# boromir674/relation-autoencoder

Hardware: AMD Instinct MI355X
Metric: train examples/sec (fwd+bwd) K=100 d=200 neg=20 at 1/2/4/8 MI355X (higher is better)
Workload: dtype fp32

## Files before the change

relation-autoencoder_amd/csrc/rae.hip:

```cpp
#include <hip/hip_runtime.h>
#include <hip/hip_ext.h>

#include <algorithm>
#include <cmath>
#include <cstdlib>
#include <cstdio>
#include <cstring>
#include <string>
#include <type_traits>

#include "../../include/rae.h"
#include "rae_bilinear.hpp"
#include "rae_cluster.hpp"
#include "rae_sp_split.hpp"
#include "rae_common.hpp"
#include "rae_dp.hpp"
#include "rae_eval.hpp"
#include "rae_index.hpp"
#include "rae_label.hpp"
#include "rae_p2p.hpp"
#include "rae_profile.hpp"
#include "rae_rank.hpp"
#include "rae_topk.hpp"
#include "rae_sampler.hpp"
// ... 493 lines not shown
    __shared__ double red[RAE_EV_NW * RAE_RK_NSUM];
    rank_blocksum(greater, equal, target, lse, n, hk, partial, red);
}
__global__ void k_rank_acc(const double* partial, int nblk, double* summary, int init) {
    const int c = threadIdx.x;
    if (blockIdx.x != 0 || c >= RAE_RK_NSUM) return;
    double t = init ? 0.0 : summary[c];
    for (int b = 0; b < nblk; ++b) t += partial[b * RAE_RK_NSUM + c];
    summary[c] = t;
}

template <bool AV4>
__global__ __launch_bounds__(RAE_RK_BT) void k_topk(RankArgs a, TopkOut o) {
    extern __shared__ __attribute__((aligned(16))) char smem[];
    topk_scores<AV4>(a, o, smem);
}
__global__ __launch_bounds__(RAE_ETK_FQ * 64) void k_topk_finish(const rae_key64* keys, int strips,
                                                                  int nq, int top, int32_t* ents,
                                                                  float* scores) {
    __shared__ rae_key64 sList[RAE_ETK_FQ * 32];
    topk_finish(keys, strips, nq, top, ents, scores, sList);
}

__global__ void k_add_cursor(int64_t* cursor, int64_t count) {
    if (threadIdx.x == 0 && blockIdx.x == 0) *cursor += count;
}
__global__ void k_set_cursor(int64_t* cursor, int64_t v) {
    if (threadIdx.x == 0 && blockIdx.x == 0) *cursor = v;
}

static thread_local std::string g_last_error;

static int fail(int code, const std::string& msg) {
    g_last_error = msg;
    return code;
}
#define HIPCHK(x)                                                                          \
    do {                                                                                   \
        hipError_t e_ = (x);                                                               \
        if (e_ != hipSuccess)                                                              \
            return fail(RAE_E_HIP, std::string(#x) + ": " + hipGetErrorString(e_));       \
    } while (0)

struct rae_plan : PlanSpec {
    rae_config cfg;
    rae_buffers buf;
    int64_t cursor_moves = 0;
    int* h_err = nullptr;
    unsigned* d_sig = nullptr;
    bool peers_set = false;
    int peers_mask = 0;
    char* ws = nullptr;
    unsigned long long* stamps_fwd = nullptr;
    unsigned long long* stamps_upd = nullptr;
    hipEvent_t t_start = nullptr, t_stop = nullptr;
};

#define RAE_LAUNCH(p, K, g, b, sh, st, ...)                                                 \
    do {                                                                                  \
        if ((p)->t_stop) {                                                                \
            hipEvent_t e0_ = (p)->t_start;                                                \
            (p)->t_start = nullptr;                                                       \
            hipExtLaunchKernelGGL(K, g, b, sh, st, e0_, (p)->t_stop, 0, __VA_ARGS__);      \
        } else {                                                                          \
            hipLaunchKernelGGL(K, g, b, sh, st, __VA_ARGS__);                             \
        }                                                                                 \
    } while (0)

#define RAE_CV(x) decltype(x)::value
template <class F> static void with_bool(bool b, F&& f) {
    if (b) f(std::true_type{}); else f(std::false_type{});
}
template <class F> static void with_q(int q, F&& f) {
    if (q == 1) f(std::integral_constant<int, 1>{}); else f(std::integral_constant<int, 2>{});
}
template <class F> static void with_opt(int opt, F&& f) {
    if (opt == RAE_OPT_ADAGRAD) f(std::integral_constant<int, 0>{});
    else f(std::integral_constant<int, 1>{});
}

extern "C" const char* rae_last_error(void) { return g_last_error.c_str(); }
extern "C" int rae_version(void) { return RAE_VERSION; }
#ifndef RAE_BUILD_ID
#define RAE_BUILD_ID "unversioned"
#endif
#ifdef RAE_DIAG
#define RAE_BUILD_KIND "diag-"
#else
#define RAE_BUILD_KIND ""
#endif
__attribute__((used)) static const char g_build_id[] = "RAE_BUILD_ID:" RAE_BUILD_KIND RAE_BUILD_ID;
extern "C" const char* rae_build_id(void) { return g_build_id + 13; }

extern "C" int64_t rae_exchange_record_floats(const rae_config* cfg) {
    if (!cfg) return -1;
    return plan_layout(*cfg).rec;
}
extern "C" int64_t rae_exchange_floats(const rae_config* cfg) {
    if (!cfg) return -1;
    return rae_exchange_record_floats(cfg) * (int64_t)cfg->batch_size * cfg->world_size;
}

static void plan_set_kernel_attributes(const rae_plan* p) {
    auto lds = [](const void* f, size_t bytes) {
        (void)hipFuncSetAttribute(f, hipFuncAttributeMaxDynamicSharedMemorySize, (int)bytes);
    };
// ... 140 lines not shown

static void launch_fwd_dp(rae_plan* p, const StepArgs& a, hipStream_t st);
template <bool V4>
static void launch_fwd_bil(rae_plan* p, const StepArgs& a, hipStream_t st) {
    const dim3 ge(p->grid_fwd);
    if (V4 && a.dec == RAE_DEC_RESCAL && a.m == 100 && a.r == 200 && a.s == 20)
        RAE_LAUNCH(p, (k_bil_enc_fast<DimsC3>), ge, dim3(RAE_FBT), p->smem_fwd, st, a);
    else
        RAE_LAUNCH(p, (k_bil_enc<V4>), ge, dim3(RAE_FBT), p->smem_fwd, st, a);
    const dim3 gmt(((a.r + RAE_MTI - 1) / RAE_MTI) * ((a.r + RAE_MTJ - 1) / RAE_MTJ));
    for (int pass = 0; pass < 2; ++pass) {
        if (pass == 1) RAE_LAUNCH(p, (k_bil_dec<V4>), ge, dim3(RAE_DBT), p->smem_dec, st, a);
        if (p->mt_bf16 && pass == 0)
            RAE_LAUNCH(p, (k_bil_mt<true, false, false>), gmt, dim3(RAE_MTT), p->smem_mt0, st, a, pass);
        else if (p->mt_bf16) RAE_LAUNCH(p, (k_bil_mt<true>), gmt, dim3(RAE_MTT), p->smem_mt, st, a, pass);
        else if (p->mt_direct) RAE_LAUNCH(p, (k_bil_mt<false, true>), gmt, dim3(RAE_MTT), 0, st, a, pass);
        else RAE_LAUNCH(p, (k_bil_mt<false>), gmt, dim3(RAE_MTT), p->smem_mt, st, a, pass);
    }
    if (!a.mtP) launch_fwd_dp(p, a, st);
    RAE_LAUNCH(p, k_bil_fin, ge, dim3(RAE_FINT), 0, st, a);
}

static void launch_fwd_dp(rae_plan* p, const StepArgs& a, hipStream_t st) {
    const int gd = ceil_div(bil_dp_tasks(a.l, a.m, a.nib), RAE_NWAVE);
    const size_t lds77 = dp2_lds_bytes<7, 7>(), lds88 = dp2_lds_bytes<8, 8>();
    if (p->dp2 == 1)
        RAE_LAUNCH(p, (k_bil_dp2<7, 7>), dim3(a.nib), dim3(dp2_threads<7, 7>()), lds77, st, a);
    else if (p->dp2 == 2)
        RAE_LAUNCH(p, (k_bil_dp2<8, 8>), dim3(a.nib), dim3(dp2_threads<8, 8>()), lds88, st, a);
    else
        with_bool(a.bf16, [&](auto B) { RAE_LAUNCH(p, k_bil_dp<RAE_CV(B)>, dim3(gd), dim3(RAE_BT), 0, st, a); });
}

static unsigned p2p_rows_grid(const StepArgs& a) {
    const int64_t g = ((int64_t)a.G * (a.capA + a.capW) + RAE_NWAVE - 1) / RAE_NWAVE;
    return (unsigned)(g < 1 ? 1 : g);
}
static unsigned p2p_recs_grid(const StepArgs& a) {
    const int64_t g = ((int64_t)a.l * a.lay.rec / 4 + RAE_BT - 1) / RAE_BT;
    return (unsigned)(g < 1 ? 1 : g);
}
static bool p2p_on(const rae_plan* p) { return p->args.xchg != RAE_XCHG_COLLECTIVE && p->args.G > 1; }
static int p2p_pre_mark_blocks(const StepArgs& a) {
    const int64_t n = (int64_t)a.G * (a.capA + a.capW);
    return (int)((n + RAE_BT - 1) / RAE_BT);
}

static int launch_forward(rae_plan* p, const int64_t* cursor, int64_t off, hipStream_t st) {
    if (!p->args.neg1 || !p->args.neg2) return fail(RAE_E_STATE, "negatives not set");
    StepArgs a = p->args;
    a.cursor = cursor;
    a.step_offset = off;
    a.stamps = p->stamps_fwd;
    const bool p2p = p2p_on(p);
    if (p2p) {
        if (!p->peers_set) return fail(RAE_E_STATE, "peer buffers not set (rae_set_peer)");
        if (!a.pipe) {
            const unsigned gr = p2p_rows_grid(a);
            RAE_LAUNCH(p, k_p2p_rows, dim3(gr), dim3(RAE_BT), 0, st, a);
            RAE_LAUNCH(p, k_p2p_signal, dim3(1), dim3(64), 0, st, a, 1);
        }
        RAE_LAUNCH(p, k_p2p_wait, dim3(1), dim3(64), 0, st, a, 1, 1u);
    }
    if (a.dec == RAE_DEC_SP) {
        launch_fwd_sp(p, a, st);
        if (a.dpart)
            RAE_LAUNCH(p, k_dpart, dim3(dpart_tasks(a.r, a.m)), dim3(RAE_BT), 0, st, a);
    }
    else with_bool(p->v4, [&](auto V) { launch_fwd_bil<RAE_CV(V)>(p, a, st); });
    if (p2p)
    {
        RAE_LAUNCH(p, k_p2p_recs, dim3(p2p_recs_grid(a) + (a.pipe ? 64 : 0)), dim3(RAE_BT), 0, st, a);
        RAE_LAUNCH(p, k_p2p_signal, dim3(1), dim3(64), 0, st, a, 0);
        if (a.pipe) {
            const int nmb = p2p_pre_mark_blocks(a);
            RAE_LAUNCH(p, k_p2p_pre, dim3(nmb + p2p_rows_grid(a)), dim3(RAE_BT), 0, st, a, 0, nmb);
        }
    }
    p->t_start = p->t_stop = nullptr;
    HIPCHK(hipGetLastError());
    return RAE_OK;
}

template <int OPT, bool V4, bool BIL>
static void launch_update_b(rae_plan* p, dim3 gu, dim3 bt, hipStream_t st, const StepArgs& a) {
    if constexpr (BIL) {
        if (a.bf16 && !a.fuse_prep) {
            const int gp = 4 * ((a.r + 63) / 64) * (a.Lp / 32) + (a.Lp / 32) * ((a.m + 15) / 16);
            RAE_LAUNCH(p, k_bil_prep, dim3(gp), bt, 0, st, a);
        }
        const int nRt = n_rtiles(a.dec, a.r, a.m);
        const dim3 gr((nRt + RAE_NWAVE - 1) / RAE_NWAVE);
        const size_t lr = bil_rows_lds_bytes(a.m, a.bf16, OPT == 0);
        constexpr size_t lu = 4 * update_lds_floats<V4, 2>();
        if (RAE_BIL_FUSED_UPD && lr >= lu) {
            const dim3 gf(gu.x + gr.x);
            with_bool(a.pipe, [&](auto PP) { with_q(p->q, [&](auto Q) {
                RAE_LAUNCH(p, (k_bil_update<OPT, V4, RAE_CV(Q), RAE_CV(PP)>), gf, bt, lr, st, a, (int)gu.x);
            }); });
            return;
        }
        with_bool(lr != 0, [&](auto LDS) {
            RAE_LAUNCH(p, (k_bil_rows<OPT, RAE_CV(LDS)>), gr, bt, lr, st, a);
        });
        with_bool(a.pipe, [&](auto PP) { with_q(p->q, [&](auto Q) {
            RAE_LAUNCH(p, (k_update_bil<OPT, V4, RAE_CV(Q), RAE_CV(PP)>), gu, bt, 0, st, a);
// ... 306 lines not shown

extern "C" int rae_time_next(rae_plan* p, void* start, void* stop) {
    if (!p) return fail(RAE_E_INVALID, "null plan");
    if (!start || !stop) return fail(RAE_E_INVALID, "null event");
    p->t_start = (hipEvent_t)start;
    p->t_stop = (hipEvent_t)stop;
    return RAE_OK;
}
extern "C" int rae_event_create(void** ev) {
    if (!ev) return fail(RAE_E_INVALID, "null argument");
    hipEvent_t e = nullptr;
    HIPCHK(hipEventCreate(&e));
    *ev = (void*)e;
    return RAE_OK;
}
extern "C" int rae_event_destroy(void* ev) {
    if (ev) HIPCHK(hipEventDestroy((hipEvent_t)ev));
    return RAE_OK;
}
extern "C" int rae_event_elapsed_ms(void* start, void* stop, float* ms) {
    if (!start || !stop || !ms) return fail(RAE_E_INVALID, "null argument");
    HIPCHK(hipEventSynchronize((hipEvent_t)stop));
    HIPCHK(hipEventElapsedTime(ms, (hipEvent_t)start, (hipEvent_t)stop));
    return RAE_OK;
}

extern "C" int rae_train_step(rae_plan* p, int64_t batch, const int32_t* n1, const int32_t* n2,
                              rae_stream_t stream) {
    if (!p) return fail(RAE_E_INVALID, "null plan");
    if (p->cfg.world_size != 1)
        return fail(RAE_E_STATE, "rae_train_step is the single-rank func['train'] path");
    const int64_t nb = p->cfg.n_examples / p->cfg.batch_size;
    if (batch < 0 || batch >= nb) return fail(RAE_E_INVALID, "batch index out of range");
    int rc = rae_set_negatives(p, n1, n2, RAE_NEG_PER_CALL, p->cfg.batch_size);
    if (rc) return rc;
    rc = launch_index(p, batch, 1, (hipStream_t)stream);
    if (rc) return rc;
    rc = launch_forward(p, nullptr, batch, (hipStream_t)stream);
    if (rc) return rc;
    return launch_update(p, nullptr, batch, (hipStream_t)stream);
}

#ifdef RAE_STAMPS
extern "C" int rae_debug_stamps(rae_plan* p, unsigned long long* buf, int fwd) {
    if (!p) return fail(RAE_E_INVALID, "null plan");
    p->stamps_fwd = fwd ? buf : nullptr;
    p->stamps_upd = fwd ? nullptr : buf;
    return RAE_OK;
}
extern "C" int rae_debug_grid(rae_plan* p, int* out) {
    out[0] = p->grid_fwd; out[1] = p->grid_update; out[2] = 0; out[3] = 0;
    return RAE_OK;
}
#endif

static int err_flags(int e) {
    if (!e) return RAE_OK;
    static const struct { int bit; const char* what; } bits[] = {
        {1, "an entity-row index partition overflowed its LDS sort"},
        {2, "a feature-row index partition overflowed its LDS sort"},
        {4, "a batch exceeded the row index's record capacity"},
        {8, "a data-parallel row list overflowed while being built"},
        {16, "a data-parallel row list is longer than the exchange's row capacity"},
        {64, "a peer-to-peer wait timed out (a peer stopped signalling)"},
    };
    std::string msg;
    for (const auto& b : bits)
        if (e & b.bit) msg += (msg.empty() ? "" : "; ") + std::string(b.what);
    msg += " (device error flags=" + std::to_string(e) + ")";
    return fail(e & 64 ? RAE_E_STATE : RAE_E_OVERFLOW, msg);
}
extern "C" int rae_check(rae_plan* p) {
    if (!p) return fail(RAE_E_INVALID, "null plan");
    int e = 0;
    HIPCHK(hipMemcpy(&e, p->d_err, sizeof(int), hipMemcpyDeviceToHost));
    return err_flags(e);
}
extern "C" int rae_check_on(rae_plan* p, rae_stream_t stream) {
    if (!p) return fail(RAE_E_INVALID, "null plan");
    HIPCHK(hipMemcpyAsync(p->h_err, p->d_err, sizeof(int), hipMemcpyDeviceToHost,
                          (hipStream_t)stream));
    HIPCHK(hipStreamSynchronize((hipStream_t)stream));
    return err_flags(*p->h_err);
}

static int launch_neg(const double* cum, int64_t n, const double* u, uint64_t seed,
                      uint64_t offset, int64_t count, int32_t* out, hipStream_t st, bool philox) {
    if (!cum || !out || (!philox && !u)) return fail(RAE_E_INVALID, "null argument");
    if (n < 1 || n >= (1ll << 31)) return fail(RAE_E_INVALID, "CDF size must be in [1, 2^31)");
    if (count <= 0) return RAE_OK;
    int64_t blocks = (count + 255) / 256;
    if (blocks > 65536) blocks = 65536;
    if (philox)
        hipLaunchKernelGGL(k_neg_sample<true>, dim3((unsigned)blocks), dim3(256), 0, st, cum, n, u,
                           seed, offset, count, out);
    else
        hipLaunchKernelGGL(k_neg_sample<false>, dim3((unsigned)blocks), dim3(256), 0, st, cum, n, u,
                           seed, offset, count, out);
    HIPCHK(hipGetLastError());
    return RAE_OK;
}

extern "C" int rae_neg_sample(const double* cum, int64_t n, const double* u, int64_t count,
                              int32_t* out, rae_stream_t stream) {
    return launch_neg(cum, n, u, 0, 0, count, out, (hipStream_t)stream, false);
}
// ... 741 lines not shown
```

relation-autoencoder_amd/csrc/rae_sp.hpp:

```cpp
#pragma once
#include "rae_common.hpp"
#include "rae_step.hpp"

namespace rae {

#define RAE_FNW (RAE_FBT / RAE_WAVE)
#define RAE_NG (RAE_FBT / 16)
#ifndef RAE_CEARLY
#define RAE_CEARLY 0
#endif

struct DynDims {
    int m, r, s;
    __device__ explicit DynDims(const StepArgs& a) : m(a.m), r(a.r), s(a.s) {}
    static constexpr bool fixed = false;
};
template <int M, int R, int S>
struct FixDims {
    static constexpr int m = M, r = R, s = S;
    __device__ explicit FixDims(const StepArgs&) {}
    static constexpr bool fixed = true;
};

template <class D> struct DimT { static constexpr int m = 0, r = 0; };
template <int M, int R, int S> struct DimT<FixDims<M, R, S>> { static constexpr int m = M, r = R; };

struct ExampleSmem {
    float *sP, *sZ, *sdP, *swC1, *swC2, *sdw1, *sdw2, *srows, *sdots, *sAbv, *scoef,
        *sred, *spart, *sfval, *sX, *sY, *sM;
    int *sfidx, *sids, *sint;
};

__host__ __device__ inline int pad_m(int m) { return ((m + 255) / 256) * 256; }

__host__ __device__ inline int example_smem_floats(int dec, int m, int r, int s) {
    const int mp = pad_m(m), r4 = align4(r), NJ = 2 + 2 * s, NJ4 = align4(NJ);
    const int NR = (dec == 0) ? 1 + 2 * s : 2 + 2 * s;
    int partf = (RAE_FNW * mp > RAE_FBT * 4) ? RAE_FNW * mp : RAE_FBT * 4;
    if (16 * r4 > partf) partf = 16 * r4;
    int f = 3 * mp + 4 * r4 + NR * r4 + 2 * NJ4 + align4(3 * NJ) + 64 + partf +
            2 * RAE_FBT + NJ4 + 16;
    if (dec != 0) f += 3 * r4 + 4 * r4;
    return f;
}

__device__ inline ExampleSmem carve_example_smem(char* smem, int dec, int m, int r, int s) {
    ExampleSmem S;
    const int mp = pad_m(m), r4 = align4(r), NJ = 2 + 2 * s, NJ4 = align4(NJ);
    const int NR = (dec == 0) ? 1 + 2 * s : 2 + 2 * s;
    int partf = (RAE_FNW * mp > RAE_FBT * 4) ? RAE_FNW * mp : RAE_FBT * 4;
    if (16 * r4 > partf) partf = 16 * r4;
    float* p = reinterpret_cast<float*>(smem);
    S.sP = p; p += mp;
    S.sZ = p; p += mp;
    S.sdP = p; p += mp;
    S.swC1 = p; p += r4;
    S.swC2 = p; p += r4;
    S.sdw1 = p; p += r4;
    S.sdw2 = p; p += r4;
    S.srows = p; p += NR * r4;
    S.sdots = p; p += NJ4;
    S.sAbv = p; p += NJ4;
    S.scoef = p; p += align4(3 * NJ);
// ... 47 lines not shown
}

typedef __attribute__((address_space(3))) void rae_lds_void;
typedef __attribute__((address_space(1))) void rae_glob_void;

template <bool V4, class D>
__device__ __forceinline__ void gather_rows_dma(const StepArgs& a, const D& Dm, ExampleSmem& S,
                                                int NR, int skip_e2, int w0 = 0,
                                                int nw = RAE_FNW) {
    constexpr int VW = V4 ? 4 : 1;
    const int lane = threadIdx.x & 63, w = (threadIdx.x >> 6) - w0;
    const int rv = Dm.r / VW, r4 = align4(Dm.r);
    const int nchunk = (rv + 63) / 64;
    for (int t = w; t < NR * nchunk; t += nw) {
        const int rho = t / nchunk, ch = t - rho * nchunk;
        const int j = (rho == 0) ? 0 : rho + skip_e2;
        const int c = ch * 64 + lane;
        float* dst = S.srows + rho * r4 + ch * 64 * VW;
        if (c < rv) {
            const float* src = a.A + (int64_t)S.sids[j] * Dm.r + (int64_t)c * VW;
            if constexpr (V4)
                __builtin_amdgcn_global_load_lds((rae_glob_void*)src, (rae_lds_void*)dst, 16, 0, 0);
            else
                __builtin_amdgcn_global_load_lds((rae_glob_void*)src, (rae_lds_void*)dst, 4, 0, 0);
        }
    }
}

#ifndef RAE_KO_C
#define RAE_KO_C 0
#endif
#ifndef RAE_KO_W
#define RAE_KO_W 0
#endif
#ifndef RAE_KO_A
#define RAE_KO_A 0
#endif
#if (RAE_KO_C || RAE_KO_W || RAE_KO_A) && !defined(RAE_DIAG)
#error "RAE_KO_C / RAE_KO_W / RAE_KO_A are timing knockouts with wrong results: a diagnostic build (-DRAE_DIAG)"
#endif

template <int VW_, class D>
struct CCacheW {
    typedef typename VecW<VW_>::T VT;
    static constexpr int VW = VW_;
    static constexpr int RA0 = D::fixed ? (DimT<D>::r + RAE_NG - 1) / RAE_NG : 7;
    static constexpr int CC0 = D::fixed ? (DimT<D>::m / VW + 15) / 16 : 2;
    static constexpr bool FITS = D::fixed && RA0 <= 7 && CC0 <= 2;
    static constexpr int RA = FITS ? RA0 : 7;
    static constexpr int CC = FITS ? CC0 : 2;
    VT c1[RA][CC], c2[RA][CC];

    __device__ __forceinline__ void load(const StepArgs& a, const D& Dm, int r0, int c0) {
        const VT* C1v = reinterpret_cast<const VT*>(a.C1);
        const VT* C2v = reinterpret_cast<const VT*>(a.C2);
        const int mv = Dm.m / VW;
        const int gid = threadIdx.x >> 4, q = threadIdx.x & 15;
#pragma unroll
        for (int ra = 0; ra < RA; ++ra) {
#if RAE_KO_C
            const int i = 0;
#else
            const int i = min(r0 + gid + RAE_NG * ra, Dm.r - 1);
#endif
#pragma unroll
            for (int cc = 0; cc < CC; ++cc) {
                const int c = min(c0 + q + 16 * cc, mv - 1);
                c1[ra][cc] = C1v[i * mv + c];
                c2[ra][cc] = C2v[i * mv + c];
            }
        }
    }
};
template <bool V4, class D> using CCache = CCacheW<V4 ? 4 : 1, D>;

template <bool V4, class D>
__device__ __forceinline__ void sp_project(const StepArgs& a, const D& Dm, ExampleSmem& S,
                                           CCache<V4, D>& cc_) {
    typedef typename VecT<V4>::T VT;
    typedef CCache<V4, D> CC_;
    const int mv = Dm.m / CC_::VW;
    const int gid = threadIdx.x >> 4, q = threadIdx.x & 15;
    const VT* Pv = reinterpret_cast<const VT*>(S.sP);
    for (int r0 = 0; r0 < Dm.r; r0 += RAE_NG * CC_::RA) {
        float s1[CC_::RA], s2[CC_::RA];
#pragma unroll
        for (int ra = 0; ra < CC_::RA; ++ra) s1[ra] = s2[ra] = 0.f;
        for (int c0 = 0; c0 < mv; c0 += 16 * CC_::CC) {
            if (!CC_::FITS) cc_.load(a, Dm, r0, c0);
#pragma unroll
            for (int cc = 0; cc < CC_::CC; ++cc) {
                const VT p = Pv[c0 + q + 16 * cc];
#pragma unroll
                for (int ra = 0; ra < CC_::RA; ++ra) {
                    s1[ra] += vdot(cc_.c1[ra][cc], p);
                    s2[ra] += vdot(cc_.c2[ra][cc], p);
                }
            }
        }
#pragma unroll
        for (int ra = 0; ra < CC_::RA; ++ra) {
            const float t1 = group16_sum(s1[ra]);
            const float t2 = group16_sum(s2[ra]);
            const int i = r0 + gid + RAE_NG * ra;
            if (q == 0 && i < Dm.r) {
                S.swC1[i] = t1;
                S.swC2[i] = t2;
            }
        }
    }
}

// ... 457 lines not shown
        sigmoid_softplus(gg, sg, spl);
        dg = sg * a.invD;
        ls = -spl;
    }
    float hs = group16_sum(dg);
    hs += __uint_as_float(xor16_u32(__float_as_uint(hs)));
    const float other = __uint_as_float(xor32_u32(__float_as_uint(hs)));
    const float sdg1 = hi ? other : hs, sdg2 = hi ? hs : other;
    const float one = left + right;
    const float u1 = one + S.sAbv[0], u2 = one + S.sAbv[1];
    float su1, spu1, su2, spu2;
    sigmoid_softplus(-u1, su1, spu1);
    sigmoid_softplus(-u2, su2, spu2);
    const float du1 = -su1 * a.invD, du2 = -su2 * a.invD;
    const float dl = du1 + du2 + sdg2;
    const float dr = du1 + du2 + sdg1;
    if (w < 2) {
        const VT* R = reinterpret_cast<const VT*>(S.srows);
        const float c0 = w == 0 ? dl : dr;
        const int off = w == 0 ? 0 : s;
        if (w == 0) {
            if (tq < s) {
                float* c = S.scoef + 3 * (2 + (hi ? s : 0) + tq);
                c[0] = hi ? 0.f : dg;
                c[1] = hi ? dg : 0.f;
                c[2] = dg;
            }
            const float sls = wave_sum(ls);
            if (lane == 0) {
                S.scoef[0] = dl; S.scoef[1] = dr; S.scoef[2] = du1;
                S.scoef[3] = 0.f; S.scoef[4] = 0.f; S.scoef[5] = du2;
                S.sred[32] = -spu1 - spu2 + 2.f * H + sls;
            }
        }
        const int lc = lane < rv ? lane : 0;
        VT v;
        vzero(v);
        vfma(v, c0, R[lc]);
        for (int t = 0; t < s; ++t) {
            const float ct = __int_as_float(__builtin_amdgcn_readlane(__float_as_int(dg),
                                                                       (w == 0 ? 0 : 32) + t));
            vfma(v, ct, R[(1 + off + t) * r4v + lc]);
        }
        if (lane < rv) reinterpret_cast<VT*>(w == 0 ? S.sdw1 : S.sdw2)[lane] = v;
    } else {
        for (int k = threadIdx.x - 2 * RAE_WAVE; k < mp; k += RAE_FBT - 2 * RAE_WAVE) S.sdP[k] = 0.f;
    }
    __syncthreads();
}

#ifndef RAE_FWD_PFLAG
#define RAE_FWD_PFLAG 1
#endif
#ifndef RAE_FWD_CWAIT
#define RAE_FWD_CWAIT 1
#endif
#ifndef RAE_FWD_CEARLY47
#define RAE_FWD_CEARLY47 0
#endif
template <bool V4, class D>
__device__ void sp_example(const StepArgs& a, int64_t g, int bl, char* smem) {
    const D Dm(a);
    const int m = Dm.m, r = Dm.r, s = Dm.s, NR = 1 + 2 * s;
    constexpr bool VR = V4 || (D::fixed && DimT<D>::r % 4 == 0);
    const int r4 = align4(r), mp = pad_m(m);
    const int lane = threadIdx.x & 63, w = threadIdx.x >> 6;
    ExampleSmem S = carve_example_smem(smem, 0, m, r, s);
    const int bg = a.rank * a.l + bl;
    const int64_t ex = g * (int64_t)a.L + bg;
    const int64_t col = a.neg_mode ? ex : (int64_t)bg;

    RAE_STAMP(a, 0);
#ifdef RAE_STAMPS
    if (a.stamps && threadIdx.x == 0) a.stamps[(size_t)blockIdx.x * 16 + 14] = __builtin_amdgcn_s_memtime();
#endif
    CCache<V4, D> cc_;
#if RAE_CEARLY
    if (CCache<V4, D>::FITS) cc_.load(a, Dm, 0, 0);
    constexpr bool kLoadC = false;
#else
    constexpr bool kLoadC = CCache<V4, D>::FITS;
#endif
    load_desc(a, Dm, g, bl, S);
    __syncthreads();
    RAE_STAMP(a, 1);
    const int NJ = 2 + 2 * s;
    if (threadIdx.x < NJ) S.sAbv[threadIdx.x] = a.Ab[S.sids[threadIdx.x]];
    encoder_forward<V4, VR, kLoadC>(a, Dm, S, NR, 1, cc_, true);
    const float H = S.sred[40];
    RAE_STAMP(a, 2);
    sp_project<V4>(a, Dm, S, cc_);
    __syncthreads();
    RAE_STAMP(a, 3);

    sp_dots<VR>(Dm, S);
    __syncthreads();
    RAE_STAMP(a, 4);

    if (s <= 32 && r / (VR ? 4 : 1) <= RAE_WAVE) {
        sp_coef_rows_regs<VR>(a, Dm, S, H);
        RAE_STAMP(a, 8);
    } else {
        sp_coefficients(a, Dm, S, H);
        __syncthreads();
        RAE_STAMP(a, 8);
        sp_weighted_rows<VR>(Dm, S);
        for (int k = threadIdx.x; k < mp; k += RAE_FBT) S.sdP[k] = 0.f;
        __syncthreads();
    }
    RAE_STAMP(a, 5);
    sp_project_back<V4>(a, Dm, S, cc_);
    RAE_STAMP(a, 9);
    softmax_backward_record(a, Dm, S, bg);
    RAE_STAMP(a, 6);
    RAE_STAMP(a, 7);
#ifdef RAE_STAMPS
    if (a.stamps && threadIdx.x == 0) a.stamps[(size_t)blockIdx.x * 16 + 15] = __builtin_amdgcn_s_memtime();
#endif
}

__device__ __forceinline__ uint32_t lds_addr(const float* p) {
    return (uint32_t)(uintptr_t)(const __attribute__((address_space(3))) float*)p;
}
__device__ __forceinline__ void dma_row16(const float* gsrc, uint32_t lds) {
    uint32_t saved;
    asm volatile("s_mov_b32 %0, m0\n\ts_mov_b32 m0, %2\n\ts_nop 0\n\t"
                 "global_load_lds_dwordx4 %1, off\n\ts_mov_b32 m0, %0"
                 : "=&s"(saved) : "v"(gsrc), "s"(lds) : "memory");
}

template <class T>
__device__ __forceinline__ void rec_st(T* p, T v) { *p = v; }

template <int m, int NSL, int NI>
__device__ __forceinline__ void fast_softmax(const StepArgs& a, ExampleSmem& S, const float (&wbk)[NI],
// ... 17 lines not shown
    float se = 0.f;
#pragma unroll
    for (int i = 0; i < NI; ++i) {
        const int k = lane + RAE_WAVE * i;
        ev[i] = k < m ? __expf(sv[i] - mx) : 0.f;
        se += ev[i];
    }
    se = wave_sum(se);
    const float inv = 1.f / se, lse = __logf(se);
    float hp = 0.f;
#pragma unroll
    for (int i = 0; i < NI; ++i) {
        const int k = lane + RAE_WAVE * i;
        const float z = k < m ? sv[i] - mx : 0.f;
        const float p = ev[i] * inv;
        S.sZ[k] = z;
        S.sP[k] = p;
        pz[i] = z;
        pp[i] = p;
        hp += p * (z - lse);
    }
    hp = wave_sum(hp);
    if (lane == 0) S.sred[40] = -a.alpha * hp;
}

template <class D> struct FastSP { static constexpr int VM = 4; static constexpr bool ok = false; };
template <int M, int R, int S> struct FastSP<FixDims<M, R, S>> {
    static constexpr int VM = M % 4 == 0 ? 4 : 2;
    static constexpr bool ok = M % 2 == 0 && R % 4 == 0 && S <= 32 && M / VM <= 32 &&
                               R / 4 <= RAE_WAVE;
};
template <class D>
__device__ void sp_example_fast(const StepArgs& a, int64_t g, int bl, char* smem) {
    static_assert(FastSP<D>::ok, "fast SP path");
    constexpr int m = D::m, r = D::r, s = D::s, NR = 1 + 2 * s, NJ = 2 + 2 * s;
    constexpr int VM = FastSP<D>::VM;
    typedef typename VecW<VM>::T MT;
    typedef CCacheW<VM, D> CCF;
    constexpr int MV = m / VM, NSL = 256 / MV, KF = 3;
    constexpr int r4 = r, mp = ((m + 255) / 256) * 256;
    const D Dm(a);
    const int tid = threadIdx.x, lane = tid & 63;
    const int w = __builtin_amdgcn_readfirstlane(tid >> 6);
    ExampleSmem S = carve_example_smem(smem, 0, m, r, s);
    float* const arows = S.srows;
    const int bg = a.rank * a.l + bl;
    const int64_t ex = g * (int64_t)a.L + bg;
    const int64_t col = a.neg_mode ? ex : (int64_t)bg;

    RAE_STAMP(a, 0);
#ifdef RAE_STAMPS
    if (a.stamps && threadIdx.x == 0) a.stamps[(size_t)blockIdx.x * 16 + 14] = __builtin_amdgcn_s_memtime();
#endif
    CCF cc_;
#if RAE_FWD_CWAIT && RAE_FWD_CEARLY47
    if (w >= 4) cc_.load(a, Dm, 0, 0);
#endif
    {
        const int32_t* dsc = a.desc + ((g % a.index_window) * a.dnx + a.d0 + bl) * (int64_t)a.dstride;
        if (tid < a.dstride) {
            const int v = dsc[tid];
            if (tid == 0) S.sint[1] = v;
            else if (tid == 1) S.sint[0] = v;
            else if (tid < 2 + NJ) S.sids[tid - 2] = v;
            else if (tid - 2 - NJ < 256) {
                S.sfidx[tid - 2 - NJ] = v;
                S.sfval[tid - 2 - NJ] = 1.f;
            }
        }
    }
    constexpr int NI = mp / RAE_WAVE;
    float wbk[NI];
#pragma unroll
    for (int i = 0; i < NI; ++i) {
        const int k = lane + RAE_WAVE * i;
        wbk[i] = (w == 0 && k < m) ? a.Wb[k] : 0.f;
    }
    if (tid == 0) {
        S.sint[4] = 0;
        S.sint[5] = 0;
    }
    lds_barrier();
    RAE_STAMP(a, 1);
    const int p0 = S.sint[0], nf = S.sint[1];
#if RAE_FWD_CWAIT
    if (nf > a.dcap || nf > NSL * KF) {
#else
    if (nf > a.dcap) {
#endif
        lds_barrier();
        sp_example<VM == 4, D>(a, g, bl, smem);
        return;
    }
    if (a.values) {
        if (w < 4 && tid < nf) S.sfval[tid] = a.values[p0 + tid];
        lds_barrier();
    }
    RAE_STAMP(a, 10);

    const MT* Wm = reinterpret_cast<const MT*>(a.W);
    const int slot = tid / MV, c = tid - slot * MV;
    MT wv[KF];
    float fv[KF];
    if (w < 4) {
#pragma unroll
        for (int k = 0; k < KF; ++k) {
            const int f = slot + NSL * k;
            const bool ok = slot < NSL && f < nf;
            const int fi = RAE_KO_W ? 0 : S.sfidx[f < 256 ? f : 255];
            wv[k] = Wm[(int64_t)(ok ? fi : 0) * MV + c];
            fv[k] = ok ? S.sfval[f < 256 ? f : 255] : 0.f;
        }
    }
    lds_barrier();
    RAE_STAMP(a, 11);
    float abv = 0.f;
#if RAE_FWD_CWAIT
    if (w >= 4) {
        static_assert(r / 4 <= RAE_WAVE, "one DMA instruction per A row");
        constexpr int RPW4 = (NR + 3) / 4;
        const int ln = lane < r / 4 ? lane : 0;
#pragma unroll
        for (int k = 0; k < RPW4; ++k) {
            const int rho = (w - 4) + 4 * k;
            if (rho < NR && lane < r / 4) {
                const int j = rho == 0 ? 0 : rho + 1;
                const float* src = a.A + (int64_t)(RAE_KO_A ? 0 : S.sids[j]) * r + (int64_t)ln * 4;
                dma_row16(src, lds_addr(arows + rho * r4));
            }
        }
        if (tid - 256 < NJ) abv = a.Ab[S.sids[tid - 256]];
    }
    asm volatile("" ::: "memory");
    if (!RAE_FWD_CEARLY47 || w < 4) cc_.load(a, Dm, 0, 0);
    if (w < 4) {
        MT acc;
        vzero(acc);
#pragma unroll
        for (int k = 0; k < KF; ++k) vfma(acc, fv[k], wv[k]);
        if (slot < NSL) reinterpret_cast<MT*>(S.spart)[slot * MV + c] = acc;
    }
    if (false) {
#else
    if (w < 4) {
#endif
        asm volatile("" ::: "memory");
        cc_.load(a, Dm, 0, 0);
        MT acc;
        vzero(acc);
#pragma unroll
        for (int k = 0; k < KF; ++k) vfma(acc, fv[k], wv[k]);
        if (slot < NSL) {
#if !RAE_FWD_CWAIT
            for (int f = slot + NSL * KF; f < nf; f += NSL)
                vfma(acc, S.sfval[f], Wm[(int64_t)S.sfidx[f] * MV + c]);
#endif
            reinterpret_cast<MT*>(S.spart)[slot * MV + c] = acc;
        }
    } else if (!RAE_FWD_CWAIT) {
        gather_rows_dma<true>(a, Dm, S, NR, 1, 4, 4);
        if (tid - 256 < NJ) abv = a.Ab[S.sids[tid - 256]];
        asm volatile("" ::: "memory");
        cc_.load(a, Dm, 0, 0);
    }
    RAE_STAMP(a, 12);
    if (w < 4) {
        asm volatile("s_waitcnt lgkmcnt(0)" ::: "memory");
        if (lane == 0) atomicAdd(&S.sint[4], 1);
    }
    if (w == 0) {
        while (__hip_atomic_load(&S.sint[4], __ATOMIC_RELAXED, __HIP_MEMORY_SCOPE_WORKGROUP) < 4)
            __builtin_amdgcn_s_sleep(1);
        RAE_STAMP(a, 13);
        float pz[NI], pp[NI];
        fast_softmax<m, NSL, NI>(a, S, wbk, lane, pz, pp);
        if (RAE_FWD_PFLAG) {
            asm volatile("s_waitcnt lgkmcnt(0)" ::: "memory");
            if (lane == 0) __hip_atomic_store(&S.sint[5], 1, __ATOMIC_RELAXED, __HIP_MEMORY_SCOPE_WORKGROUP);
        }
    }
    if (RAE_FWD_PFLAG) {
        if (w != 0)
            while (__hip_atomic_load(&S.sint[5], __ATOMIC_RELAXED, __HIP_MEMORY_SCOPE_WORKGROUP) == 0)
                __builtin_amdgcn_s_sleep(1);
        asm volatile("" ::: "memory");
    } else {
        lds_barrier();
    }
    const float H = S.sred[40];
    RAE_STAMP(a, 2);
#if RAE_FWD_CWAIT
    {
        typedef CCF CC_;
        static_assert(CC_::FITS && CC_::CC <= 2, "fast path keeps C1/C2 in registers");
        const int gid = tid >> 4, q = tid & 15;
        const MT* Pv = reinterpret_cast<const MT*>(S.sP);
        MT pv[CC_::CC];
#pragma unroll
        for (int cc = 0; cc < CC_::CC; ++cc) pv[cc] = Pv[q + 16 * cc];
        float s1[CC_::RA], s2[CC_::RA];
#pragma unroll
        for (int ra = 0; ra < CC_::RA; ++ra) {
            s1[ra] = vdot(cc_.c1[ra][0], pv[0]);
            s2[ra] = vdot(cc_.c2[ra][0], pv[0]);
#pragma unroll
            for (int cc = 1; cc < CC_::CC; ++cc) {
                s1[ra] += vdot(cc_.c1[ra][cc], pv[cc]);
                s2[ra] += vdot(cc_.c2[ra][cc], pv[cc]);
            }
        }
#pragma unroll
        for (int ra = 0; ra < CC_::RA; ++ra) {
            s1[ra] = group16_sum(s1[ra]);
            s2[ra] = group16_sum(s2[ra]);
        }
        if (q == 0) {
#pragma unroll
            for (int ra = 0; ra < CC_::RA; ++ra) {
                const int i = gid + RAE_NG * ra;
                if (i < r) {
                    S.swC1[i] = s1[ra];
                    S.swC2[i] = s2[ra];
                }
            }
        }
    }
#else
    sp_project<true>(a, Dm, S, cc_);
#endif
    if (w >= 4 && tid - 256 < NJ) S.sAbv[tid - 256] = abv;
    dma_visible_barrier();
    RAE_STAMP(a, 3);

    constexpr int RV = r / 4;
    static_assert(RV <= RAE_WAVE, "one float4 column per lane");
    const bool lv = lane < RV;
    const float4 z4 = make_float4(0.f, 0.f, 0.f, 0.f);
    const float4* Rv = reinterpret_cast<const float4*>(arows);
    const int lc = lv ? lane : 0;
    float4 wc1 = reinterpret_cast<const float4*>(S.swC1)[lc];
    float4 wc2 = reinterpret_cast<const float4*>(S.swC2)[lc];
    if (!lv) wc1 = wc2 = z4;
    {
        constexpr int RPW = (NR + RAE_FNW - 1) / RAE_FNW;
        float d[RPW];
        float4 xr[RPW];
#pragma unroll
        for (int q = 0; q < RPW; ++q) {
            const int rho = w + RAE_FNW * q;
            xr[q] = Rv[(rho < NR ? rho : 0) * RV + lc];
        }
#pragma unroll
        for (int q = 0; q < RPW; ++q) {
            const int rho = w + RAE_FNW * q;
            const float v = vdot(xr[q], rho > s ? wc2 : wc1);
            d[q] = rho < NR ? v : 0.f;
        }
        float d0b = (w == 0) ? vdot(xr[0], wc2) : 0.f;
#pragma unroll
        for (int q = 0; q < RPW; ++q) d[q] = wave_sum(d[q]);
        if (w == 0) d0b = wave_sum(d0b);
        if (lane == 0) {
#pragma unroll
            for (int q = 0; q < RPW; ++q) {
                const int rho = w + RAE_FNW * q;
                if (rho == 0) {
                    S.sdots[0] = d[q];
                    S.sdots[1] = d0b;
                } else if (rho < NR) {
                    S.sdots[rho + 1] = d[q];
                }
            }
        }
    }
    lds_barrier();
    RAE_STAMP(a, 4);

    const float left = S.sdots[0], right = S.sdots[1];
    const int tq = lane & 31;
    const bool hi = lane >= 32;
    float dg = 0.f, ls = 0.f;
    if (tq < s) {
// ... 119 lines not shown
                if (col < MV) S.spart[w * mp + 4 * col + e] = t[cc];
            }
        } else {
#pragma unroll
            for (int cc = 0; cc < CC_::CC; ++cc) {
                float* v = reinterpret_cast<float*>(&acc[cc]);
#pragma unroll
                for (int e = 0; e < VM; ++e) {
                    v[e] += __uint_as_float(xor16_u32(__float_as_uint(v[e])));
                    v[e] += __uint_as_float(xor32_u32(__float_as_uint(v[e])));
                }
                const int col = q + 16 * cc;
                if (lane < 16 && col < MV) reinterpret_cast<MT*>(S.spart + w * mp)[col] = acc[cc];
            }
        }
    }
    lds_barrier();
    RAE_STAMP(a, 9);

    if (w == 0) {
        const float ce = 2.f * a.alpha * a.invD;
        float pk[NI], zk[NI], dp[NI];
        float sd = 0.f, sz = 0.f;
#pragma unroll
        for (int i = 0; i < NI; ++i) {
            const int k = lane + RAE_WAVE * i;
            float v = 0.f;
            if (k < m) {
#pragma unroll
                for (int ww = 0; ww < RAE_FNW; ++ww) v += S.spart[ww * mp + k];
            }
            dp[i] = v;
            pk[i] = k < m ? S.sP[k] : 0.f;
            zk[i] = k < m ? S.sZ[k] : 0.f;
            sd += pk[i] * dp[i];
            sz += pk[i] * zk[i];
        }
        sd = wave_sum(sd);
        sz = wave_sum(sz);
#pragma unroll
        for (int i = 0; i < NI; ++i) {
            const int k = lane + RAE_WAVE * i;
            if (k < m) {
                rec_st(rec + a.lay.oP + k, pk[i]);
                rec_st(rec + a.lay.odS + k, pk[i] * ((dp[i] - sd) + ce * (zk[i] - sz)));
            }
        }
    }
    RAE_STAMP(a, 6);
    RAE_STAMP(a, 7);
#ifdef RAE_STAMPS
    if (a.stamps && threadIdx.x == 0) a.stamps[(size_t)blockIdx.x * 16 + 15] = __builtin_amdgcn_s_memtime();
#endif
}


}
```

relation-autoencoder_amd/csrc/rae_step.hpp:

```cpp
#pragma once
#include <stdint.h>

namespace rae {

struct RecLayout {
    int oP, odS, oV1, oV2, odw1, odw2, oG1, ocoef, oloss, rec;
    int oG2, oX, oY, oA1, oA2, oZ, oAux;
    int wire;
    int oPart, pc;
};

__host__ __device__ inline int align4(int x) { return (x + 3) & ~3; }

__host__ __device__ inline int dense_partial_floats(int r, int m) { return 2 * r * m + m; }

__host__ __device__ inline RecLayout make_layout(int dec, int m, int r, int s, int wire = 0,
                                                 int l = 1) {
    RecLayout L{};
    const int NJ = 2 + 2 * s;
    const int m4 = align4(m), r4 = align4(r);
    L.oP = 0;
    L.odS = m4;
    L.oPart = -1;
    if (dec == 0 && wire) {
// ... 83 lines not shown
    int VCA, VCW;
    int32_t *thdr, *task, *vtask;
    int TC, NVC;
    int hch, HF, hps;
    float* hpart;
    int32_t* hfin;
    int32_t* desc;
    int dstride, dcap;
    int dnx, d0;
    const int64_t* cursor;
    int64_t step_offset;
    float* costs;
    float* gWs;
    float* dPpart;
    float* sps;
    int spss;
    float* mtV;
    float* mtW;
    float* mtP;
    int nmtp;
    int r4;
    int nib;
    int bf16;
    float* facT;
    uint4* pfrag;
    int Lp;
    int fuse_prep;
    double* regpart;
    int nregC;
    int nregW;
    float* base_cost;
    int* err;
    int G, part;
    int32_t* dpl;
    int32_t* dpc;
    int LA, LW;
    float* dsend;
    float* drecv;
    int capA, capW;
    int64_t dblk;
    int* dpmax;
    int xchg;
    PeerBufs* peers;
    unsigned* sig;
    unsigned* p2p_expect;
    unsigned long long p2p_timeout;
    int pipe;
    uint32_t* pm;
    int pmA, pmW;
    int priv, privnf;
    int privc;
    int32_t* pmask;
    unsigned long long* stamps;
};

__device__ __forceinline__ int64_t step_batch(const StepArgs& a) {
    return a.cursor ? *a.cursor + a.step_offset : a.step_offset;
}

#if defined(RAE_DIAG_NOSINGLE) && !defined(RAE_DIAG)
#error "RAE_DIAG_NOSINGLE is a timing knockout with wrong results: a diagnostic build (-DRAE_DIAG)"
#endif
#if defined(RAE_STAMPS) && !defined(RAE_DIAG)
#error "RAE_STAMPS instruments the kernels for tools/phase_stamps.py: a diagnostic build (-DRAE_DIAG)"
#endif
#ifdef RAE_STAMPS
#define RAE_STAMP(a, slot)                                                                  \
    do {                                                                                    \
        if ((a).stamps && threadIdx.x == 0)                                                 \
            (a).stamps[(size_t)blockIdx.x * 16 + (slot)] = __builtin_amdgcn_s_memrealtime(); \
    } while (0)
#else
#define RAE_STAMP(a, slot) do { } while (0)
#endif

}
```

Baseline: 5.877 million.

## Split forward warp roles and start C1/C2 register loads before descriptor barrier

Restructures the sparse fast-path forward so waves 4-7 begin loading part of the C1/C2 register cache before the descriptor barrier, then issue the A-row DMAs, and only then load the remaining C rows. Waves 0-3 read the descriptor, gather and reduce W, and run the softmax, with explicit vmcnt waits. The aim is to hide C-cache load latency behind the descriptor fetch and the W gather when C1/C2 exceed a size threshold. It also removes the old CWAIT/CEARLY compile variants and adds optional per-wave timestamp instrumentation for diagnostic builds. Early loads raise register pressure, and the reordered barriers risk subtle synchronization mistakes.

```diff
diff --git a/relation-autoencoder_amd/csrc/rae.hip b/relation-autoencoder_amd/csrc/rae.hip
--- a/relation-autoencoder_amd/csrc/rae.hip
+++ b/relation-autoencoder_amd/csrc/rae.hip
@@ -569,6 +569,9 @@
     int peers_mask = 0;
     char* ws = nullptr;
     unsigned long long* stamps_fwd = nullptr;
+#ifdef RAE_WSTAMPS
+    unsigned long long* stamps_wave = nullptr;
+#endif
     unsigned long long* stamps_upd = nullptr;
     hipEvent_t t_start = nullptr, t_stop = nullptr;
 };
@@ -815,6 +818,9 @@
     a.cursor = cursor;
     a.step_offset = off;
     a.stamps = p->stamps_fwd;
+#ifdef RAE_WSTAMPS
+    a.wstamps = p->stamps_wave;
+#endif
     const bool p2p = p2p_on(p);
     if (p2p) {
         if (!p->peers_set) return fail(RAE_E_STATE, "peer buffers not set (rae_set_peer)");
@@ -1227,6 +1233,13 @@
     out[0] = p->grid_fwd; out[1] = p->grid_update; out[2] = 0; out[3] = 0;
     return RAE_OK;
 }
+#ifdef RAE_WSTAMPS
+extern "C" int rae_debug_wave_stamps(rae_plan* p, unsigned long long* buf) {
+    if (!p) return fail(RAE_E_INVALID, "null plan");
+    p->stamps_wave = buf;
+    return RAE_OK;
+}
+#endif
 #endif
 
 static int err_flags(int e) {
diff --git a/relation-autoencoder_amd/csrc/rae_sp.hpp b/relation-autoencoder_amd/csrc/rae_sp.hpp
--- a/relation-autoencoder_amd/csrc/rae_sp.hpp
+++ b/relation-autoencoder_amd/csrc/rae_sp.hpp
@@ -6,9 +6,6 @@
 
 #define RAE_FNW (RAE_FBT / RAE_WAVE)
 #define RAE_NG (RAE_FBT / 16)
-#ifndef RAE_CEARLY
-#define RAE_CEARLY 0
-#endif
 
 struct DynDims {
     int m, r, s;
@@ -162,12 +159,17 @@
     VT c1[RA][CC], c2[RA][CC];
 
     __device__ __forceinline__ void load(const StepArgs& a, const D& Dm, int r0, int c0) {
+        load_rows<0, RA>(a, Dm, r0, c0);
+    }
+    template <int RA_B, int RA_E>
+    __device__ __forceinline__ void load_rows(const StepArgs& a, const D& Dm, int r0, int c0) {
+        static_assert(0 <= RA_B && RA_B <= RA_E && RA_E <= RA, "row-group range");
         const VT* C1v = reinterpret_cast<const VT*>(a.C1);
         const VT* C2v = reinterpret_cast<const VT*>(a.C2);
         const int mv = Dm.m / VW;
         const int gid = threadIdx.x >> 4, q = threadIdx.x & 15;
 #pragma unroll
-        for (int ra = 0; ra < RA; ++ra) {
+        for (int ra = RA_B; ra < RA_E; ++ra) {
 #if RAE_KO_C
             const int i = 0;
 #else
@@ -731,11 +733,19 @@
 #ifndef RAE_FWD_PFLAG
 #define RAE_FWD_PFLAG 1
 #endif
-#ifndef RAE_FWD_CWAIT
-#define RAE_FWD_CWAIT 1
-#endif
-#ifndef RAE_FWD_CEARLY47
-#define RAE_FWD_CEARLY47 0
+#ifndef RAE_FWD_CE47
+#define RAE_FWD_CE47 7
+#endif
+#define RAE_WAIT_VM0 0x0F70
+#if defined(RAE_WSTAMPS) && !defined(RAE_STAMPS)
+#error "RAE_WSTAMPS extends RAE_STAMPS (a diagnostic build)"
+#endif
+#ifdef RAE_WSTAMPS
+#define RAE_WSTAMP_T(k) (wst[k] = __builtin_amdgcn_s_memrealtime())
+#define RAE_WSTAMP_WAIT(n) asm volatile("s_waitcnt vmcnt(%0)" ::"n"(n) : "memory")
+#else
+#define RAE_WSTAMP_T(k) do { } while (0)
+#define RAE_WSTAMP_WAIT(n) do { } while (0)
 #endif
 template <bool V4, class D>
 __device__ void sp_example(const StepArgs& a, int64_t g, int bl, char* smem) {
@@ -754,12 +764,7 @@
     if (a.stamps && threadIdx.x == 0) a.stamps[(size_t)blockIdx.x * 16 + 14] = __builtin_amdgcn_s_memtime();
 #endif
     CCache<V4, D> cc_;
-#if RAE_CEARLY
-    if (CCache<V4, D>::FITS) cc_.load(a, Dm, 0, 0);
-    constexpr bool kLoadC = false;
-#else
     constexpr bool kLoadC = CCache<V4, D>::FITS;
-#endif
     load_desc(a, Dm, g, bl, S);
     __syncthreads();
     RAE_STAMP(a, 1);
@@ -883,147 +888,157 @@
 #ifdef RAE_STAMPS
     if (a.stamps && threadIdx.x == 0) a.stamps[(size_t)blockIdx.x * 16 + 14] = __builtin_amdgcn_s_memtime();
 #endif
+#ifdef RAE_WSTAMPS
+    unsigned long long wst[8] = {0, 0, 0, 0, 0, 0, 0, 0};
+#endif
+    RAE_WSTAMP_T(0);
     CCF cc_;
-#if RAE_FWD_CWAIT && RAE_FWD_CEARLY47
-    if (w >= 4) cc_.load(a, Dm, 0, 0);
-#endif
-    {
+    constexpr bool kEarly = 2 * r * m * (int)sizeof(float) > 32 * 1024;
+    constexpr int E47 = !kEarly ? 0 : RAE_FWD_CE47 < CCF::RA ? RAE_FWD_CE47 : CCF::RA;
+    constexpr int NI = mp / RAE_WAVE;
+    static_assert(CCF::FITS && CCF::CC <= 2, "fast path keeps C1/C2 in registers");
+    static_assert(r / 4 <= RAE_WAVE, "one DMA instruction per A row");
+    float abv = 0.f;
+    bool general;
+    if (w >= 4) {
+        cc_.template load_rows<0, E47>(a, Dm, 0, 0);
+        RAE_WSTAMP_T(1);
+        lds_barrier();
+        const int nf = S.sint[1];
+        general = nf > a.dcap || nf > NSL * KF;
+        if (!general) {
+            if (a.values) lds_barrier();
+            lds_barrier();
+            constexpr int RPW4 = (NR + 3) / 4;
+            const int ln = lane < r / 4 ? lane : 0;
+#pragma unroll
+            for (int k = 0; k < RPW4; ++k) {
+                const int rho = (w - 4) + 4 * k;
+                if (rho < NR && lane < r / 4) {
+                    const int j = rho == 0 ? 0 : rho + 1;
+                    const float* src = a.A + (int64_t)(RAE_KO_A ? 0 : S.sids[j]) * r + (int64_t)ln * 4;
+                    dma_row16(src, lds_addr(arows + rho * r4));
+                }
+            }
+        }
+        if (tid - 256 < NJ) abv = a.Ab[S.sids[tid - 256]];
+        asm volatile("" ::: "memory");
+        cc_.template load_rows<E47, CCF::RA>(a, Dm, 0, 0);
+        asm volatile("" ::: "memory");
+        RAE_WSTAMP_T(2);
+        if (!general) {
+#ifdef RAE_WSTAMPS
+            RAE_WSTAMP_WAIT((CCF::RA - E47) * CCF::CC * 2);
+            RAE_WSTAMP_T(3);
+            RAE_WSTAMP_WAIT(0);
+            RAE_WSTAMP_T(4);
+#endif
+            if (RAE_FWD_PFLAG) {
+                while (__hip_atomic_load(&S.sint[5], __ATOMIC_RELAXED, __HIP_MEMORY_SCOPE_WORKGROUP) == 0)
+                    __builtin_amdgcn_s_sleep(1);
+            } else {
+                lds_barrier();
+            }
+        }
+    } else {
+        constexpr int DN = 2 + NJ + NSL * KF;
+        static_assert(DN <= 4 * RAE_WAVE, "the descriptor read is waves 0-3's");
         const int32_t* dsc = a.desc + ((g % a.index_window) * a.dnx + a.d0 + bl) * (int64_t)a.dstride;
-        if (tid < a.dstride) {
+        if (tid < DN && tid < a.dstride) {
             const int v = dsc[tid];
             if (tid == 0) S.sint[1] = v;
             else if (tid == 1) S.sint[0] = v;
             else if (tid < 2 + NJ) S.sids[tid - 2] = v;
-            else if (tid - 2 - NJ < 256) {
+            else {
                 S.sfidx[tid - 2 - NJ] = v;
                 S.sfval[tid - 2 - NJ] = 1.f;
             }
         }
-    }
-    constexpr int NI = mp / RAE_WAVE;
-    float wbk[NI];
-#pragma unroll
-    for (int i = 0; i < NI; ++i) {
-        const int k = lane + RAE_WAVE * i;
-        wbk[i] = (w == 0 && k < m) ? a.Wb[k] : 0.f;
-    }
-    if (tid == 0) {
-        S.sint[4] = 0;
-        S.sint[5] = 0;
-    }
-    lds_barrier();
-    RAE_STAMP(a, 1);
-    const int p0 = S.sint[0], nf = S.sint[1];
-#if RAE_FWD_CWAIT
-    if (nf > a.dcap || nf > NSL * KF) {
-#else
-    if (nf > a.dcap) {
-#endif
+        if (tid == 0) {
+            S.sint[4] = 0;
+            S.sint[5] = 0;
+        }
+        __builtin_amdgcn_s_waitcnt(RAE_WAIT_VM0);
+        RAE_WSTAMP_T(1);
+        lds_barrier();
+        RAE_STAMP(a, 1);
+        const int p0 = S.sint[0], nf = S.sint[1];
+        general = nf > a.dcap || nf > NSL * KF;
+        if (!general) {
+            if (a.values) {
+                if (tid < nf) S.sfval[tid] = a.values[p0 + tid];
+                __builtin_amdgcn_s_waitcnt(RAE_WAIT_VM0);
+                lds_barrier();
+            }
+            RAE_STAMP(a, 10);
+            const MT* Wm = reinterpret_cast<const MT*>(a.W);
+            const int slot = tid / MV, c = tid - slot * MV;
+            MT wv[KF];
+            float fv[KF];
+#pragma unroll
+            for (int k = 0; k < KF; ++k) {
+                const int f = slot + NSL * k;
+                const bool ok = slot < NSL && f < nf;
+                const int fi = RAE_KO_W ? 0 : S.sfidx[f < 256 ? f : 255];
+                wv[k] = Wm[(int64_t)(ok ? fi : 0) * MV + c];
+                fv[k] = ok ? S.sfval[f < 256 ? f : 255] : 0.f;
+            }
+            float wbk[NI];
+#pragma unroll
+            for (int i = 0; i < NI; ++i) {
+                const int k = lane + RAE_WAVE * i;
+                wbk[i] = (w == 0 && k < m) ? a.Wb[k] : 0.f;
+            }
+            lds_barrier();
+            RAE_STAMP(a, 11);
+            asm volatile("" ::: "memory");
+            cc_.template load_rows<0, CCF::RA>(a, Dm, 0, 0);
+            RAE_WSTAMP_T(2);
+            {
+                MT acc;
+                vzero(acc);
+#pragma unroll
+                for (int k = 0; k < KF; ++k) vfma(acc, fv[k], wv[k]);
+                if (slot < NSL) reinterpret_cast<MT*>(S.spart)[slot * MV + c] = acc;
+            }
+            RAE_WSTAMP_T(3);
+            RAE_STAMP(a, 12);
+            asm volatile("s_waitcnt lgkmcnt(0)" ::: "memory");
+            if (lane == 0) atomicAdd(&S.sint[4], 1);
+            if (w == 0) {
+                while (__hip_atomic_load(&S.sint[4], __ATOMIC_RELAXED, __HIP_MEMORY_SCOPE_WORKGROUP) < 4)
+                    __builtin_amdgcn_s_sleep(1);
+                RAE_STAMP(a, 13);
+                float pz[NI], pp[NI];
+                fast_softmax<m, NSL, NI>(a, S, wbk, lane, pz, pp);
+                if (RAE_FWD_PFLAG) {
+                    asm volatile("s_waitcnt lgkmcnt(0)" ::: "memory");
+                    if (lane == 0) __hip_atomic_store(&S.sint[5], 1, __ATOMIC_RELAXED, __HIP_MEMORY_SCOPE_WORKGROUP);
+                }
+            } else {
+#ifdef RAE_WSTAMPS
+                RAE_WSTAMP_WAIT(0);
+                RAE_WSTAMP_T(4);
+#endif
+                if (RAE_FWD_PFLAG)
+                    while (__hip_atomic_load(&S.sint[5], __ATOMIC_RELAXED, __HIP_MEMORY_SCOPE_WORKGROUP) == 0)
+                        __builtin_amdgcn_s_sleep(1);
+            }
+            if (!RAE_FWD_PFLAG) lds_barrier();
+        }
+    }
+    if (general) {
+        __builtin_amdgcn_s_waitcnt(RAE_WAIT_VM0);
         lds_barrier();
         sp_example<VM == 4, D>(a, g, bl, smem);
         return;
     }
-    if (a.values) {
-        if (w < 4 && tid < nf) S.sfval[tid] = a.values[p0 + tid];
-        lds_barrier();
-    }
-    RAE_STAMP(a, 10);
-
-    const MT* Wm = reinterpret_cast<const MT*>(a.W);
-    const int slot = tid / MV, c = tid - slot * MV;
-    MT wv[KF];
-    float fv[KF];
-    if (w < 4) {
-#pragma unroll
-        for (int k = 0; k < KF; ++k) {
-            const int f = slot + NSL * k;
-            const bool ok = slot < NSL && f < nf;
-            const int fi = RAE_KO_W ? 0 : S.sfidx[f < 256 ? f : 255];
-            wv[k] = Wm[(int64_t)(ok ? fi : 0) * MV + c];
-            fv[k] = ok ? S.sfval[f < 256 ? f : 255] : 0.f;
-        }
-    }
-    lds_barrier();
-    RAE_STAMP(a, 11);
-    float abv = 0.f;
-#if RAE_FWD_CWAIT
-    if (w >= 4) {
-        static_assert(r / 4 <= RAE_WAVE, "one DMA instruction per A row");
-        constexpr int RPW4 = (NR + 3) / 4;
-        const int ln = lane < r / 4 ? lane : 0;
-#pragma unroll
-        for (int k = 0; k < RPW4; ++k) {
-            const int rho = (w - 4) + 4 * k;
-            if (rho < NR && lane < r / 4) {
-                const int j = rho == 0 ? 0 : rho + 1;
-                const float* src = a.A + (int64_t)(RAE_KO_A ? 0 : S.sids[j]) * r + (int64_t)ln * 4;
-                dma_row16(src, lds_addr(arows + rho * r4));
-            }
-        }
-        if (tid - 256 < NJ) abv = a.Ab[S.sids[tid - 256]];
-    }
     asm volatile("" ::: "memory");
-    if (!RAE_FWD_CEARLY47 || w < 4) cc_.load(a, Dm, 0, 0);
-    if (w < 4) {
-        MT acc;
-        vzero(acc);
-#pragma unroll
-        for (int k = 0; k < KF; ++k) vfma(acc, fv[k], wv[k]);
-        if (slot < NSL) reinterpret_cast<MT*>(S.spart)[slot * MV + c] = acc;
-    }
-    if (false) {
-#else
-    if (w < 4) {
-#endif
-        asm volatile("" ::: "memory");
-        cc_.load(a, Dm, 0, 0);
-        MT acc;
-        vzero(acc);
-#pragma unroll
-        for (int k = 0; k < KF; ++k) vfma(acc, fv[k], wv[k]);
-        if (slot < NSL) {
-#if !RAE_FWD_CWAIT
-            for (int f = slot + NSL * KF; f < nf; f += NSL)
-                vfma(acc, S.sfval[f], Wm[(int64_t)S.sfidx[f] * MV + c]);
-#endif
-            reinterpret_cast<MT*>(S.spart)[slot * MV + c] = acc;
-        }
-    } else if (!RAE_FWD_CWAIT) {
-        gather_rows_dma<true>(a, Dm, S, NR, 1, 4, 4);
-        if (tid - 256 < NJ) abv = a.Ab[S.sids[tid - 256]];
-        asm volatile("" ::: "memory");
-        cc_.load(a, Dm, 0, 0);
-    }
-    RAE_STAMP(a, 12);
-    if (w < 4) {
-        asm volatile("s_waitcnt lgkmcnt(0)" ::: "memory");
-        if (lane == 0) atomicAdd(&S.sint[4], 1);
-    }
-    if (w == 0) {
-        while (__hip_atomic_load(&S.sint[4], __ATOMIC_RELAXED, __HIP_MEMORY_SCOPE_WORKGROUP) < 4)
-            __builtin_amdgcn_s_sleep(1);
-        RAE_STAMP(a, 13);
-        float pz[NI], pp[NI];
-        fast_softmax<m, NSL, NI>(a, S, wbk, lane, pz, pp);
-        if (RAE_FWD_PFLAG) {
-            asm volatile("s_waitcnt lgkmcnt(0)" ::: "memory");
-            if (lane == 0) __hip_atomic_store(&S.sint[5], 1, __ATOMIC_RELAXED, __HIP_MEMORY_SCOPE_WORKGROUP);
-        }
-    }
-    if (RAE_FWD_PFLAG) {
-        if (w != 0)
-            while (__hip_atomic_load(&S.sint[5], __ATOMIC_RELAXED, __HIP_MEMORY_SCOPE_WORKGROUP) == 0)
-                __builtin_amdgcn_s_sleep(1);
-        asm volatile("" ::: "memory");
-    } else {
-        lds_barrier();
-    }
     const float H = S.sred[40];
     RAE_STAMP(a, 2);
-#if RAE_FWD_CWAIT
+    RAE_WSTAMP_T(5);
     {
         typedef CCF CC_;
-        static_assert(CC_::FITS && CC_::CC <= 2, "fast path keeps C1/C2 in registers");
         const int gid = tid >> 4, q = tid & 15;
         const MT* Pv = reinterpret_cast<const MT*>(S.sP);
         MT pv[CC_::CC];
@@ -1056,9 +1071,7 @@
             }
         }
     }
-#else
-    sp_project<true>(a, Dm, S, cc_);
-#endif
+    RAE_WSTAMP_T(6);
     if (w >= 4 && tid - 256 < NJ) S.sAbv[tid - 256] = abv;
     dma_visible_barrier();
     RAE_STAMP(a, 3);
@@ -1284,7 +1297,15 @@
 #ifdef RAE_STAMPS
     if (a.stamps && threadIdx.x == 0) a.stamps[(size_t)blockIdx.x * 16 + 15] = __builtin_amdgcn_s_memtime();
 #endif
-}
-
-
-}
+#ifdef RAE_WSTAMPS
+    RAE_WSTAMP_T(7);
+    if (a.wstamps && lane == 0) {
+        unsigned long long* o = a.wstamps + ((size_t)blockIdx.x * RAE_FNW + w) * 8;
+#pragma unroll
+        for (int k = 0; k < 8; ++k) o[k] = wst[k];
+    }
+#endif
+}
+
+
+}
diff --git a/relation-autoencoder_amd/csrc/rae_step.hpp b/relation-autoencoder_amd/csrc/rae_step.hpp
--- a/relation-autoencoder_amd/csrc/rae_step.hpp
+++ b/relation-autoencoder_amd/csrc/rae_step.hpp
@@ -159,6 +159,9 @@
     int privc;
     int32_t* pmask;
     unsigned long long* stamps;
+#ifdef RAE_WSTAMPS
+    unsigned long long* wstamps;
+#endif
 };
 
 __device__ __forceinline__ int64_t step_batch(const StepArgs& a) {
```

Result: faster. 6.091 million, median of 6 (+3.6%).
